# VachaLab/gorder

Measured on AMD Instinct MI355X. Metric: trajectory frames/sec, higher is better.
Workload: dtype f32

## Files before the change

gorder_amd/csrc/gorder_hip.hip:

```cpp
#include <hip/hip_runtime.h>

#include <dlfcn.h>

#include <cmath>
#include <cstdio>
#include <cstdlib>
#include <cstring>
#include <mutex>
#include <new>
#include <string>
#include <deque>
#include <vector>

#include "../../include/gorder_hip.h"
#include "gm_math.h"
#include "plan.h"

#pragma clang fp contract(off)

using gorder::DirectItem;
using gorder::Item;
using gorder::kBlock;
using gorder::Plan;
using gorder::Tile;
// ... 1004 lines not shown
            for (uint32_t k = 0; k < mt.n_molecules; k++) {
                const uint32_t hd = mt.heads ? mt.heads[k] : 0;
                if (hd >= t->n_atoms) return fail(h, GORDER_ERR_INVALID_ARGUMENT, "head index out of range");
                heads.push_back(hd);
                if (lf.method == GORDER_LEAFLETS_INDIVIDUAL)
                    for (uint32_t q = 0; q < mt.n_methyls; q++) {
                        const uint32_t a = mt.methyls[(size_t)k * mt.n_methyls + q];
                        if (a >= t->n_atoms) return fail(h, GORDER_ERR_INVALID_ARGUMENT, "methyl index out of range");
                        ma.push_back(a);
                    }
                mb.push_back((uint32_t)ma.size());
            }
        }
        if ((st = upload(h, &h->d_heads, heads)) != GORDER_OK) return st;
        h->host_heads = heads;
        if (lf.method == GORDER_LEAFLETS_LOCAL) {
            std::vector<uint32_t> ms;
            for (uint32_t m = 0; m < t->n_molecule_types; m++) ms.insert(ms.end(), t->molecule_types[m].n_molecules, p.slot0[m]);
            if ((st = upload(h, &h->d_mol_slot0, ms)) != GORDER_OK) return st;
        }
        if ((st = upload(h, &h->d_methyl_begin, mb)) != GORDER_OK) return st;
        if ((st = upload(h, &h->d_methyl_atoms, ma)) != GORDER_OK) return st;
        if (lf.method == GORDER_LEAFLETS_LOCAL && !(lf.radius > 0.0f))
            return fail(h, GORDER_ERR_INVALID_ARGUMENT, "local leaflets need a positive radius");
        if (lf.method == GORDER_LEAFLETS_GLOBAL || lf.method == GORDER_LEAFLETS_LOCAL) {
            if (!lf.membrane || lf.n_membrane == 0)
                return fail(h, GORDER_ERR_INVALID_ARGUMENT, "global/local leaflets need the membrane group");
            std::vector<uint32_t> mem(lf.membrane, lf.membrane + lf.n_membrane);
            for (uint32_t a : mem)
                if (a >= t->n_atoms) return fail(h, GORDER_ERR_INVALID_ARGUMENT, "membrane index out of range");
            if ((st = upload(h, &h->d_membrane, mem)) != GORDER_OK) return st;
            h->membrane_is_frame = lf.n_membrane == t->n_atoms && !env_flag("GORDER_HIP_LEAFLETS_GENERIC");
            for (uint32_t i = 0; i < lf.n_membrane && h->membrane_is_frame; i++) h->membrane_is_frame = mem[i] == i;
        }
        if (lf.method == GORDER_LEAFLETS_GLOBAL && p.spec_ok && !env_flag("GORDER_HIP_NO_SPECULATE")) {
            std::vector<uint2> own(p.tiles.size());
            for (size_t i = 0; i < own.size(); i++) own[i] = make_uint2(p.own[2 * i], p.own[2 * i + 1]);
            if ((st = upload(h, &h->d_own, own)) != GORDER_OK) return st;
            std::vector<std::vector<SpecSample>> per_mol(p.n_mol_total);
            for (const Tile &tile : p.tiles)
                for (uint32_t q = 0; q < tile.n_items; q++) {
                    const Item &it = p.items[tile.item0 + q];
                    per_mol[it.mol].push_back({tile.atom0 + it.li, tile.atom0 + it.lj, p.tile_slots[tile.slot0 + it.lslot]});
                }
            std::vector<uint32_t> mbeg(1, 0);
            std::vector<SpecSample> all;
            for (const auto &v : per_mol) { all.insert(all.end(), v.begin(), v.end()); mbeg.push_back((uint32_t)all.size()); }
            if ((st = upload(h, &h->d_spec_mol_begin, mbeg)) != GORDER_OK) return st;
            if ((st = upload(h, &h->d_spec_samples, all)) != GORDER_OK) return st;
            std::vector<uint2> oh(p.own_heads.size() / 2);
            for (size_t i = 0; i < oh.size(); i++) oh[i] = make_uint2(p.own_heads[2 * i], p.own_heads[2 * i + 1]);
            if ((st = upload(h, &h->d_own_head_begin, p.own_head_begin)) != GORDER_OK) return st;
            if ((st = upload(h, &h->d_own_heads, oh)) != GORDER_OK) return st;
            HIP_TRY(h, hipMalloc((void **)&h->d_spec_counters, 4 * sizeof(uint32_t)));
            HIP_TRY(h, hipMemset(h->d_spec_counters, 0, 4 * sizeof(uint32_t)));
            HIP_TRY(h, hipHostMalloc((void **)&h->h_spec_counters, 2 * gorder_hip_handle::kSpecRing * sizeof(uint32_t)));
            for (hipEvent_t &ev : h->spec_counters_copied) HIP_TRY(h, hipEventCreateWithFlags(&ev, hipEventDisableTiming));
            h->spec_enabled = true;
        }
        if (lf.method == GORDER_LEAFLETS_LOCAL) {
            const size_t nm = lf.n_membrane, ncell = (size_t)kLocalMaxCells1D * kLocalMaxCells1D;
            const size_t sl = h->local_slab = local_slab_frames(nm);
            for (const void *fn : {reinterpret_cast<const void *>(k_local_build<2>), reinterpret_cast<const void *>(k_local_build<5>),
                                   reinterpret_cast<const void *>(k_local_build<kLocalBuildTrips>)})
                HIP_TRY(h, hipFuncSetAttribute(fn, hipFuncAttributeMaxDynamicSharedMemorySize, (int)kLocalBuildLds));
            h->local_halo = t->handle_pbc && !env_flag("GORDER_HIP_LOCAL_ATOMS_ONLY");
            h->local_rec_stride = (h->local_halo ? 2u : 1u) * nm;
            HIP_TRY(h, hipMalloc((void **)&h->d_lcell_of, sl * nm * sizeof(uint32_t)));
            HIP_TRY(h, hipMalloc((void **)&h->d_ltrig, sl * h->local_rec_stride * sizeof(LocalRec)));
            HIP_TRY(h, hipMalloc((void **)&h->d_lcell_count, sl * (ncell + 1) * sizeof(uint32_t)));
            HIP_TRY(h, hipMalloc((void **)&h->d_lcell_fill, sl * ncell * sizeof(uint32_t)));
            HIP_TRY(h, hipMalloc((void **)&h->d_lgrid, sl * sizeof(uint4)));
            if (h->local_halo) {
                HIP_TRY(h, hipMalloc((void **)&h->d_lrowpre, sl * (size_t)kLocalMaxCells1D * (kLocalMaxCells1D + 1u) * sizeof(LocalRowPre)));
                HIP_TRY(h, hipMalloc((void **)&h->d_ledge, sl * (size_t)kLocalMaxCells1D * (kLocalMaxCells1D + 1u) * sizeof(LocalEdge)));
                HIP_TRY(h, hipMalloc((void **)&h->d_lfinfo, sl * sizeof(float4)));
                HIP_TRY(h, hipMalloc((void **)&h->d_lneed, (sl + 1) * sizeof(uint32_t)));
                HIP_TRY(h, hipMalloc((void **)&h->d_lsummary, 2 * sizeof(uint32_t)));
                HIP_TRY(h, hipMemset(h->d_lsummary, 0, 2 * sizeof(uint32_t)));
                HIP_TRY(h, hipHostMalloc((void **)&h->h_lsummary, 2 * sizeof(uint32_t)));
                h->h_lsummary[0] = h->h_lsummary[1] = 0u;
                HIP_TRY(h, hipEventCreateWithFlags(&h->lsummary_written, hipEventDisableTiming));
                HIP_TRY(h, hipFuncSetAttribute(reinterpret_cast<const void *>(k_local_decide), hipFuncAttributeMaxDynamicSharedMemorySize,
                                               (int)kDecideLds));
                HIP_TRY(h, hipFuncSetAttribute(reinterpret_cast<const void *>(k_local_sums), hipFuncAttributeMaxDynamicSharedMemorySize,
                                               (int)kSumsLds));
                HIP_TRY(h, hipMalloc((void **)&h->d_ltodo, (1 + sl * (size_t)(p.n_mol_total ? p.n_mol_total : 1)) * sizeof(uint2)));
            }
        }
        HIP_TRY(h, hipMalloc((void **)&h->d_adist, sizeof(float) * (p.n_mol_total ? p.n_mol_total : 1)));
    }
    HIP_TRY(h, hipDeviceSynchronize());
    return GORDER_OK;
}

void gorder_hip_destroy(gorder_hip_handle *h) {
    if (!h) return;
    (void)hipSetDevice(h->device);
    if (h->stream) (void)hipStreamSynchronize(h->stream);
    if (h->traj_cache_free) h->traj_cache_free(h);
    for (hipEvent_t ev : h->timing_ev)
        if (ev) (void)hipEventDestroy(ev);
    (void)hipFree(h->d_mol_slot0);
    (void)hipFree(h->d_tiles); (void)hipFree(h->d_items); (void)hipFree(h->d_tile_slots);
    (void)hipFree(h->d_direct); (void)hipFree(h->d_err); (void)hipFree(h->d_xtc_cp);
    (void)hipFree(h->d_ua_tiles); (void)hipFree(h->d_ua_items); (void)hipFree(h->d_ua_tile_slots);
    (void)hipFree(h->d_map_sums); (void)hipFree(h->d_map_cnts); (void)hipFree(h->d_map_packed); (void)hipFree(h->d_tw_sums); (void)hipFree(h->d_tw_cnts);
    (void)hipFree(h->d_geom_group); (void)hipFree(h->d_shapes); (void)hipFree(h->d_inv_box);
// ... 38 lines not shown
    h->stream = hip_stream ? (hipStream_t)hip_stream : h->own_stream;
    return GORDER_OK;
}

static void spec_poll(gorder_hip_handle *h, bool wait);
int gorder_hip_speculation_stats(gorder_hip_handle *h, uint64_t out[4]) {
    if (!h || !out) return GORDER_ERR_INVALID_ARGUMENT;
    HIP_TRY(h, hipSetDevice(h->device));
    HIP_TRY(h, hipStreamSynchronize(h->stream));
    spec_poll(h, true);
    out[0] = h->spec_batches; out[1] = h->spec_fixed; out[2] = h->spec_exact_frames; out[3] = h->spec_enabled ? 1 : 0;
    return GORDER_OK;
}

int gorder_hip_local_decide_stats(gorder_hip_handle *h, uint64_t out[4]) {
    if (!h || !out) return GORDER_ERR_INVALID_ARGUMENT;
    HIP_TRY(h, hipSetDevice(h->device));
    HIP_TRY(h, hipStreamSynchronize(h->stream));
    out[0] = h->decide_submits; out[1] = h->decide_paused_submits;
    out[2] = h->h_lsummary ? h->h_lsummary[0] : 0; out[3] = h->h_lsummary ? h->h_lsummary[1] : 0;
    return GORDER_OK;
}

int gorder_hip_plan(const gorder_hip_handle *h, gorder_hip_plan_t *plan) {
    if (!h || !plan) return GORDER_ERR_INVALID_ARGUMENT;
    plan->n_tiles = (uint32_t)h->plan.tiles.size();
    plan->block_threads = kBlock;
    plan->max_window_atoms = h->plan.max_window;
    plan->n_direct_items = (uint32_t)h->plan.direct.size();
    plan->frames_per_stage = (uint32_t)h->frames_per_stage;
    plan->lds_bytes = (uint32_t)h->lds_bytes;
    plan->map_staged = h->map_staged ? 1u : 0u;
    plan->map_lds_bytes = (uint32_t)h->map_lds_bytes;
    plan->leaflets_one_read = h->plan.spec_ok ? 1u : 0u;
    return GORDER_OK;
}

static void spec_poll(gorder_hip_handle *h, bool wait) {
    for (uint32_t i = 0; i < gorder_hip_handle::kSpecRing; i++) {
        if (!h->spec_ring_frames[i]) continue;
        if (wait) (void)hipEventSynchronize(h->spec_counters_copied[i]);
        else if (hipEventQuery(h->spec_counters_copied[i]) != hipSuccess) continue;
        const uint32_t moved = h->h_spec_counters[2 * i], exact = h->h_spec_counters[2 * i + 1];
        h->spec_fixed += moved;
        h->spec_exact_frames += exact;
        if ((uint64_t)exact * 8u > h->spec_ring_frames[i] ||
            (uint64_t)moved * 16u > h->spec_ring_frames[i] * h->plan.n_mol_total)
            h->spec_enabled = false;
        h->spec_ring_frames[i] = 0;
    }
}

static int run_leaflets(gorder_hip_handle *h, const float *d_xyz, const float *d_box,
                        const std::vector<uint32_t> &aframes, uint32_t row0, const uint8_t *skip = nullptr) {
    if (aframes.empty()) return GORDER_OK;
    int st;
    const size_t cap_before = h->aframes_cap;
    if ((st = ensure(h, &h->d_aframes, &h->aframes_cap, aframes.size())) != GORDER_OK) return st;
    if (h->aframes_cap != cap_before) h->up_aframes_at = nullptr;
    if (h->up_aframes_at != h->d_aframes || h->up_aframes != aframes) {
        HIP_TRY(h, hipMemcpyAsync(h->d_aframes, aframes.data(), aframes.size() * sizeof(uint32_t),
                                  hipMemcpyHostToDevice, h->stream));
        h->up_aframes = aframes;
        h->up_aframes_at = h->d_aframes;
    }
    const gorder_leaflets_t &lf = h->tables.leaflets;
    LeafletArgs la{};
    la.xyz = d_xyz; la.box9 = d_box; la.n_atoms = h->plan.n_atoms;
    la.aframes = h->d_aframes; la.row0 = row0; la.aflags = h->d_aflags; la.adist = h->d_adist;
    la.n_mol_total = h->plan.n_mol_total; la.heads = h->d_heads;
    la.membrane = h->d_membrane; la.n_membrane = lf.n_membrane;
    la.methyl_begin = h->d_methyl_begin; la.methyl_atoms = h->d_methyl_atoms;
    la.dim = lf.normal_dim; la.flip = lf.flip ? 1 : 0; la.pbc = h->tables.handle_pbc ? 1 : 0;
    la.err = h->d_err;
    la.skip = skip;
    la.n_assign = (uint32_t)aframes.size();
    if (lf.method == GORDER_LEAFLETS_GLOBAL) {
        const dim3 g(skip ? std::min<uint32_t>((uint32_t)aframes.size(), 512u) : (uint32_t)aframes.size()), b(1024);
        TIMING_MARK(h, h->membrane_is_frame ? "k_leaflets_global_contig" : "k_leaflets_global");
        if (h->membrane_is_frame) {
            if (skip) hipLaunchKernelGGL(k_leaflets_global_contig<true>, g, dim3(256), 0, h->stream, la);
            else hipLaunchKernelGGL(k_leaflets_global_contig<false>, g, dim3(256), 0, h->stream, la);
        } else {
            if (skip) hipLaunchKernelGGL(k_leaflets_global<true>, g, b, 0, h->stream, la);
            else hipLaunchKernelGGL(k_leaflets_global<false>, g, b, 0, h->stream, la);
        }
    } else if (lf.method == GORDER_LEAFLETS_INDIVIDUAL) {
        TIMING_MARK(h, "k_leaflets_individual");
        size_t done = 0;
        while (done < aframes.size()) {
            const uint32_t ny = (uint32_t)std::min<size_t>(aframes.size() - done, 65535);
            LeafletArgs lb = la;
            lb.aframes = h->d_aframes + done;
            lb.row0 = row0 + (uint32_t)done;
            if (done + ny < aframes.size()) lb.adist = nullptr;
            hipLaunchKernelGGL(k_leaflets_individual, dim3((la.n_mol_total + 255) / 256, ny), dim3(256), 0,
                               h->stream, lb);
            done += ny;
        }
    }
    else if (lf.method == GORDER_LEAFLETS_LOCAL) {
        const size_t ncell = (size_t)kLocalMaxCells1D * kLocalMaxCells1D;
        LocalArgs lo{};
        lo.xyz = d_xyz; lo.box9 = d_box; lo.n_atoms = h->plan.n_atoms;
        lo.aflags = h->d_aflags; lo.adist = h->d_adist; lo.n_mol_total = h->plan.n_mol_total;
        lo.heads = h->d_heads; lo.mol_slot0 = h->d_mol_slot0; lo.n_membrane = lf.n_membrane;
        lo.membrane = h->membrane_is_frame ? nullptr : h->d_membrane;
        lo.dim = lf.normal_dim; lo.flip = lf.flip ? 1 : 0; lo.pbc = h->tables.handle_pbc ? 1 : 0;
        lo.radius = lf.radius;
        lo.radius_thr = local_radius_threshold(lf.radius);
        lo.cell_of = h->d_lcell_of; lo.trig = h->d_ltrig; lo.cell_count = h->d_lcell_count;
        lo.cell_fill = h->d_lcell_fill; lo.err = h->d_err;
        lo.grid = h->d_lgrid;
        lo.halo = h->local_halo ? 1 : 0;
        lo.prune = env_flag("GORDER_HIP_LOCAL_NO_PRUNE") ? 0 : (env_flag("GORDER_HIP_LOCAL_DECIDE_NOTHING") ? 2 : 1);
        lo.rec_stride = (uint32_t)h->local_rec_stride;
        lo.rowpre = h->d_lrowpre;
        lo.edge = h->d_ledge;
        lo.finfo = h->d_lfinfo;
        lo.todo = h->d_ltodo;
        bool decide = lo.halo && lo.prune && lo.n_mol_total && !env_flag("GORDER_HIP_LOCAL_NO_DECIDE");
        if (decide) {
            if (h->lsummary_pending) {
                if (hipEventQuery(h->lsummary_written) == hipSuccess) {
                    h->lsummary_pending = false;
                    if (2u * h->h_lsummary[0] > h->h_lsummary[1]) h->decide_pause = gorder_hip_handle::kDecidePause;
                } else {
                    (void)hipGetLastError();
// ... 145 lines not shown
        HIP_TRY(h, hipMemsetAsync(nc, 0, ncap * row * sizeof(unsigned long long), h->stream));
        if (h->d_tw_sums) {
            HIP_TRY(h, hipMemcpyAsync(ns, h->d_tw_sums, h->n_frames * row * sizeof(unsigned long long), hipMemcpyDeviceToDevice, h->stream));
            HIP_TRY(h, hipMemcpyAsync(nc, h->d_tw_cnts, h->n_frames * row * sizeof(unsigned long long), hipMemcpyDeviceToDevice, h->stream));
            HIP_TRY(h, hipStreamSynchronize(h->stream));
            HIP_TRY(h, hipFree(h->d_tw_sums));
            HIP_TRY(h, hipFree(h->d_tw_cnts));
        }
        h->d_tw_sums = ns; h->d_tw_cnts = nc; h->tw_cap = ncap;
    }
    FrameArgs a{};
    a.xyz = d_xyz; a.box9 = d_box; a.n_atoms = p.n_atoms; a.n_frames = n_frames;
    a.pbc = pbc ? 1 : 0;
    a.nx = h->tables.normal[0]; a.ny = h->tables.normal[1]; a.nz = h->tables.normal[2]; a.n2 = h->n2; a.n2sq = h->n2sq;
    a.leaflets = leaflets ? 1 : 0; a.aflags = h->d_aflags; a.arow = h->d_arow; a.n_mol_total = p.n_mol_total;
    a.acc = h->d_acc; a.rep = h->d_rep; a.n_rep = h->n_rep; a.n_acc = p.n_acc; a.err = h->d_err;
    h->manual_active = false;
    if (h->manual_frames) {
        const size_t n4 = (size_t)n_frames * p.n_mol_total;
        if ((st = ensure(h, &h->d_dyn_normals, &h->dyn_normals_cap, n4)) != GORDER_OK) return abort_batch(st);
        if (hipStreamSynchronize(h->stream) != hipSuccess ||
            hipMemcpy(h->d_dyn_normals, h->manual_normals.data(), n4 * 4 * sizeof(float), hipMemcpyHostToDevice) != hipSuccess)
            return abort_batch(fail(h, GORDER_ERR_DEVICE, "manual normals: copy to the device failed"));
        h->manual_active = true;
        h->manual_frames = 0;
    }
    const uint32_t n_tiles_all = (uint32_t)p.tiles.size();
    if (spec) {
        if ((st = ensure(h, &h->d_mom, &h->mom_cap, (size_t)n_frames * n_tiles_all)) != GORDER_OK) return abort_batch(st);
        if ((st = ensure(h, &h->d_head_z, &h->head_z_cap, (size_t)n_frames * p.n_mol_total)) != GORDER_OK) return abort_batch(st);
        a.own = h->d_own; a.mom = h->d_mom; a.mom_dim = (int)lf.normal_dim;
        a.own_head_begin = h->d_own_head_begin; a.own_heads = h->d_own_heads; a.head_z = h->d_head_z;
        h->spec_now = true;
    }
    st = launch_orders(h, a);
    h->spec_now = false;
    h->manual_active = false;
    if (st != GORDER_OK) return abort_batch(st);
    h->rep_dirty = true;
    if (spec) {
        size_t cap_c = h->spec_frames_cap, cap_o = h->spec_frames_cap;
        if ((st = ensure(h, &h->d_spec_center, &cap_c, n_frames)) != GORDER_OK) return abort_batch(st);
        if ((st = ensure(h, &h->d_spec_ok, &cap_o, n_frames)) != GORDER_OK) return abort_batch(st);
        h->spec_frames_cap = std::min(cap_c, cap_o);
        uint32_t *cnt = h->d_spec_counters + 2u * (uint32_t)(h->spec_batches & 1u);
        uint32_t *cnt_next = h->d_spec_counters + 2u * (uint32_t)((h->spec_batches + 1u) & 1u);
        SpecArgs sa{};
        sa.xyz = d_xyz; sa.box9 = d_box; sa.n_atoms = p.n_atoms; sa.n_frames = n_frames; sa.n_tiles = n_tiles_all;
        sa.n_mol_total = p.n_mol_total; sa.n_membrane = lf.n_membrane; sa.dim = lf.normal_dim; sa.flip = lf.flip ? 1 : 0;
        sa.pbc = pbc ? 1 : 0; sa.mom = h->d_mom; sa.head_z = h->d_head_z; sa.center = h->d_spec_center; sa.ok = h->d_spec_ok;
        sa.aflags = h->d_aflags; sa.adist = h->d_adist; sa.counters = cnt; sa.counters_next = cnt_next;
        const uint32_t ring_slot = (uint32_t)(h->spec_batches % gorder_hip_handle::kSpecRing);
        sa.host_counters = h->h_spec_counters + 2u * ring_slot; sa.err = h->d_err;
        (void)timing_mark(h, "k_spec_check + k_spec_fixup");
        hipLaunchKernelGGL(k_spec_check, dim3(std::min<uint32_t>(n_frames, 2048u)), dim3(256), 0, h->stream, sa);
        if ((st = run_leaflets(h, d_xyz, d_box, spec_aframes, 1, h->d_spec_ok)) != GORDER_OK) return abort_batch(st);
        (void)timing_mark(h, "k_spec_check + k_spec_fixup");
        const uint32_t fix_grid = (uint32_t)std::min<uint64_t>(((uint64_t)n_frames * p.n_mol_total + 63u) / 64u, 4096u);
        if (h->extra.tw)
            hipLaunchKernelGGL((k_spec_fixup<false, true>), dim3(fix_grid), dim3(64), 0, h->stream, a, sa, h->d_spec_mol_begin,
                               h->d_spec_samples, h->d_tw_sums, h->d_tw_cnts, (uint64_t)h->n_frames);
        else if (h->tables.flags & GORDER_FLAG_TRIG_ACOS_COS)
            hipLaunchKernelGGL((k_spec_fixup<true, false>), dim3(fix_grid), dim3(64), 0, h->stream, a, sa, h->d_spec_mol_begin,
                               h->d_spec_samples, (unsigned long long *)nullptr, (unsigned long long *)nullptr, (uint64_t)0);
        else
            hipLaunchKernelGGL((k_spec_fixup<false, false>), dim3(fix_grid), dim3(64), 0, h->stream, a, sa, h->d_spec_mol_begin,
                               h->d_spec_samples, (unsigned long long *)nullptr, (unsigned long long *)nullptr, (uint64_t)0);
        hipLaunchKernelGGL(k_spec_finish, dim3(1), dim3(256), 0, h->stream, sa);
        HIP_TRY(h, hipGetLastError());
        HIP_TRY(h, hipEventRecord(h->spec_counters_copied[ring_slot], h->stream));
        h->spec_ring_frames[ring_slot] = n_frames;
        h->spec_batches++;
    }
    if (n_new_rows) {
        HIP_TRY(h, hipMemcpyAsync(h->d_aflags, h->d_aflags + n_new_rows * (size_t)p.n_mol_total, p.n_mol_total,
                                  hipMemcpyDeviceToDevice, h->stream));
    }
    {
        gorder_hip_handle::BatchLog rec{h->n_submits, frame_index[0], n_frames > 1 ? frame_index[1] - frame_index[0] : 0, {}};
        for (uint32_t f = 1; f < n_frames; f++)
            if (frame_index[f] != rec.first + (uint64_t)f * rec.stride) { rec.list.assign(frame_index, frame_index + n_frames); break; }
        if (h->batch_log.size() >= gorder_hip_handle::kBatchLog) h->batch_log.pop_front();
        h->batch_log.push_back(std::move(rec));
        TIMING_MARK(h, "k_batch_end");
        hipLaunchKernelGGL(k_batch_end, dim3(pbc ? std::min<uint32_t>((n_frames + 255u) / 256u, 256u) : 1u), dim3(256), 0, h->stream,
                           pbc ? d_box : nullptr, n_frames, h->d_err,
                           h->d_acc + 4 * (size_t)p.n_acc, (unsigned long long)h->n_submits, h->decoder_key);
        HIP_TRY(h, hipGetLastError());
        TIMING_MARK(h, nullptr);
        if (h->timing_on) h->timing_launches++;
        h->n_submits++;
    }
    h->n_frames += n_frames;
    return GORDER_OK;
}

int gorder_hip_submit_host(gorder_hip_handle *h, const float *xyz, const float *box, const uint64_t *frame_index,
                           uint32_t n_frames) {
    if (!h || !xyz || !frame_index) return GORDER_ERR_INVALID_ARGUMENT;
    if (n_frames == 0) return GORDER_OK;
    HIP_TRY(h, hipSetDevice(h->device));
    int st;
    const size_t nx = (size_t)n_frames * h->plan.n_atoms * 3u, nb = (size_t)n_frames * 9u;
    if (!h->copy_stream) {
        HIP_TRY(h, hipStreamCreateWithFlags(&h->copy_stream, hipStreamNonBlocking));
        for (int k = 0; k < 2; k++) {
            HIP_TRY(h, hipEventCreateWithFlags(&h->stage_copied[k], hipEventDisableTiming));
            HIP_TRY(h, hipEventCreateWithFlags(&h->stage_computed[k], hipEventDisableTiming));
        }
    }
    const int b = h->stage_next;
    h->stage_next ^= 1;
    if (h->stage_used[b]) HIP_TRY(h, hipEventSynchronize(h->stage_computed[b]));
    if ((st = ensure(h, &h->d_stage_xyz[b], &h->stage_xyz_cap[b], nx)) != GORDER_OK) return st;
    HIP_TRY(h, hipMemcpyAsync(h->d_stage_xyz[b], xyz, nx * sizeof(float), hipMemcpyHostToDevice, h->copy_stream));
    if (box) {
        if ((st = ensure(h, &h->d_stage_box[b], &h->stage_box_cap[b], nb)) != GORDER_OK) return st;
        HIP_TRY(h, hipMemcpyAsync(h->d_stage_box[b], box, nb * sizeof(float), hipMemcpyHostToDevice, h->copy_stream));
    }
    HIP_TRY(h, hipEventRecord(h->stage_copied[b], h->copy_stream));
    HIP_TRY(h, hipStreamWaitEvent(h->stream, h->stage_copied[b], 0));
// ... 180 lines not shown
    HIP_TRY(h, hipMemcpyAsync(d_sums, h->d_map_sums, n * sizeof(unsigned long long), hipMemcpyDeviceToDevice, h->stream));
    HIP_TRY(h, hipMemcpyAsync(d_counts, h->d_map_cnts, n * sizeof(unsigned long long), hipMemcpyDeviceToDevice, h->stream));
    HIP_TRY(h, hipStreamSynchronize(h->stream));
    return check_device_error(h);
}

int gorder_hip_bind_accumulators(gorder_hip_handle *h, void *d_ptr, uint64_t n_u64) {
    if (!h || !d_ptr || n_u64 < h->acc_words || ((uintptr_t)d_ptr & 7u)) return GORDER_ERR_INVALID_ARGUMENT;
    HIP_TRY(h, hipSetDevice(h->device));
    {
        const int st = fold_replicas(h);
        if (st != GORDER_OK) return st;
    }
    HIP_TRY(h, hipMemcpyAsync(d_ptr, h->d_acc, h->acc_words * sizeof(unsigned long long), hipMemcpyDeviceToDevice, h->stream));
    HIP_TRY(h, hipStreamSynchronize(h->stream));
    if (!h->acc_external) HIP_TRY(h, hipFree(h->d_acc));
    h->d_acc = (unsigned long long *)d_ptr;
    h->acc_external = true;
    return GORDER_OK;
}

int gorder_hip_reset(gorder_hip_handle *h) {
    if (!h) return GORDER_ERR_INVALID_ARGUMENT;
    HIP_TRY(h, hipSetDevice(h->device));
    const Plan &p = h->plan;
    HIP_TRY(h, hipMemsetAsync(h->d_acc, 0, h->acc_words * sizeof(unsigned long long), h->stream));
    if (h->d_rep) HIP_TRY(h, hipMemsetAsync(h->d_rep, 0, (size_t)h->n_rep * 4u * p.n_acc * sizeof(unsigned long long), h->stream));
    h->rep_dirty = false;
    if (h->extra.maps) {
        const size_t nmap = 3 * (size_t)p.n_acc * h->map_nx * h->map_ny;
        const size_t npk = (h->tables.leaflets.method != GORDER_LEAFLETS_NONE ? 2 : 1) * (nmap / 3);
        HIP_TRY(h, hipMemsetAsync(h->d_map_sums, 0, nmap * sizeof(unsigned long long), h->stream));
        HIP_TRY(h, hipMemsetAsync(h->d_map_cnts, 0, nmap * sizeof(unsigned long long), h->stream));
        HIP_TRY(h, hipMemsetAsync(h->d_map_packed, 0, npk * sizeof(unsigned long long), h->stream));
        h->map_pending = 0;
    }
    if (h->d_tw_sums) {
        const size_t n = h->tw_cap * 3 * (size_t)p.n_acc * sizeof(unsigned long long);
        HIP_TRY(h, hipMemsetAsync(h->d_tw_sums, 0, n, h->stream));
        HIP_TRY(h, hipMemsetAsync(h->d_tw_cnts, 0, n, h->stream));
    }
    HIP_TRY(h, hipMemsetAsync(h->d_err, 0xff, kErrWords * sizeof(uint32_t), h->stream));
    h->batch_log.clear();
    h->n_frames = 0;
    h->have_assignment = false;
    h->assignment_frame = 0;
    h->manual_frames = 0;
    h->err_index = 0;
    h->err_msg.clear();
    if (h->d_own) {
        spec_poll(h, true);
        h->spec_enabled = true;
        h->spec_batches = h->spec_fixed = h->spec_exact_frames = 0;
        HIP_TRY(h, hipMemsetAsync(h->d_spec_counters, 0, 4 * sizeof(uint32_t), h->stream));
    }
    if (h->d_lsummary) {
        if (h->lsummary_pending) { (void)hipEventSynchronize(h->lsummary_written); h->lsummary_pending = false; }
        h->decide_pause = 0;
        h->decide_submits = h->decide_paused_submits = 0;
        h->h_lsummary[0] = h->h_lsummary[1] = 0u;
        HIP_TRY(h, hipMemsetAsync(h->d_lsummary, 0, 2 * sizeof(uint32_t), h->stream));
    }
    return GORDER_OK;
}

int gorder_hip_comm_unique_id(uint8_t id[128]) {
    if (!id) return GORDER_ERR_INVALID_ARGUMENT;
    RcclApi *api = rccl_api(nullptr);
    if (!api) return GORDER_ERR_DEVICE;
    UniqueId u;
    if (api->get_unique_id(&u) != 0) return GORDER_ERR_DEVICE;
    memcpy(id, u.internal, 128);
    return GORDER_OK;
}

int gorder_hip_comm_create(gorder_hip_handle *h, const uint8_t id[128], int n_ranks, int rank, void **comm_out) {
    if (!h || !id || !comm_out || n_ranks < 1 || rank < 0 || rank >= n_ranks) return GORDER_ERR_INVALID_ARGUMENT;
    *comm_out = nullptr;
    std::string why;
    RcclApi *api = rccl_api(&why);
    if (!api) return fail(h, GORDER_ERR_DEVICE, why);
    HIP_TRY(h, hipSetDevice(h->device));
    UniqueId u;
    memcpy(u.internal, id, 128);
    const int rc = api->comm_init_rank(comm_out, n_ranks, u, rank);
    if (rc != 0) return fail(h, GORDER_ERR_DEVICE, rccl_error(api, "ncclCommInitRank", rc));
    return GORDER_OK;
}

void gorder_hip_comm_destroy(void *comm) {
    RcclApi *api = rccl_api(nullptr);
    if (api && comm) (void)api->comm_destroy(comm);
}

int gorder_hip_allreduce(gorder_hip_handle *h, void *nccl_comm) {
    if (!h || !nccl_comm) return GORDER_ERR_INVALID_ARGUMENT;
    std::string why;
    RcclApi *api = rccl_api(&why);
    if (!api) return fail(h, GORDER_ERR_DEVICE, why);
    HIP_TRY(h, hipSetDevice(h->device));
    int st = fold_replicas(h);
    if (st != GORDER_OK) return st;
    if ((st = fold_maps(h)) != GORDER_OK) return st;
    int rc = api->group_start();
    if (rc == 0) rc = api->all_reduce(h->d_acc, h->d_acc, h->acc_words, kNcclInt64, kNcclSum, nccl_comm, h->stream);
    if (rc == 0 && h->extra.maps) {
        const size_t nmap = 3 * (size_t)h->plan.n_acc * h->map_nx * h->map_ny;
// ... 90 lines not shown
```

gorder_amd/csrc/kernels_leaflets.h:

```cpp
#pragma once

namespace {

struct LeafletArgs {
    const float *xyz;
    const float *box9;
    uint32_t n_atoms;
    const uint32_t *aframes;
    uint32_t row0;
    uint8_t *aflags;
    float *adist;
    uint32_t n_mol_total;
    const uint32_t *heads;
    const uint32_t *membrane;
    uint32_t n_membrane;
    const uint32_t *methyl_begin;
    const uint32_t *methyl_atoms;
    uint32_t dim;
    int flip, pbc;
    uint32_t *err;
    const uint8_t *skip;
    uint32_t n_assign;
};

__device__ __forceinline__ void fast_sincos_rev(float u, float *sn, float *cs);
__device__ __forceinline__ void local_trig(float z, float inv_L, float *sn, float *cs) {
    fast_sincos_rev(z * inv_L, sn, cs);
}
__device__ __forceinline__ void fast_sincos_rev(float u, float *sn, float *cs) {
    *sn = __builtin_amdgcn_sinf(u);
    *cs = __builtin_amdgcn_cosf(u);
}

__device__ __forceinline__ double wave_sum(double v) {
    for (int off = 32; off > 0; off >>= 1) v += __shfl_xor(v, off, 64);
    return v;
}

__device__ __forceinline__ double block_sum(double v, double *scratch) {
    v = wave_sum(v);
    const uint32_t wave = threadIdx.x >> 6, n_waves = (blockDim.x + 63u) >> 6;
    if ((threadIdx.x & 63u) == 0) scratch[wave] = v;
    __syncthreads();
    double r = 0.0;
    for (uint32_t w = 0; w < n_waves; w++) r += scratch[w];
    __syncthreads();
    return r;
}

__device__ __forceinline__ void block_sum2(double &v0, double &v1, double *scratch) {
    v0 = wave_sum(v0);
    v1 = wave_sum(v1);
    const uint32_t wave = threadIdx.x >> 6, n_waves = (blockDim.x + 63u) >> 6;
    if ((threadIdx.x & 63u) == 0) { scratch[wave] = v0; scratch[16 + wave] = v1; }
    __syncthreads();
    double r0 = 0.0, r1 = 0.0;
    for (uint32_t w = 0; w < n_waves; w++) { r0 += scratch[w]; r1 += scratch[16 + w]; }
    __syncthreads();
    v0 = r0; v1 = r1;
}

struct GeomArgs {
    const float *xyz;
    const float *box9;
    uint32_t n_atoms;
    int pbc;
    uint32_t kind, reference, orientation;
    float point[3];
    const uint32_t *group;
    uint32_t n_group;
    float xdim[2], ydim[2], zdim[2], radius, span[2], structure_box[3];
    float *shapes;
    uint32_t *err;
};

// ... 109 lines not shown
            float sn, cs;
            fast_sincos_rev(gm_wrap(dn == 0 ? px : (dn == 1 ? py : pz), L, bad) * inv, &sn, &cs);
            sc += cs;
            ss += sn;
        }
    }
    if (a.pbc) {
        const double tc = block_sum((double)sc, scratch), ts = block_sum((double)ss, scratch);
        est = (atan2f(-(float)ts, -(float)tc) + 3.1415927f) / (6.2831855f / L);
    }
    float acc = 0.0f;
#pragma unroll
    for (int k = 0; k < KEEP; k++) {
        const uint32_t i = threadIdx.x + (uint32_t)k * nthr;
        if (i < a.n_membrane) {
            const float dx = keep[k] - est;
            acc += a.pbc ? gm_min_image(dx, L, bad) : dx;
        }
    }
    for (uint32_t i = threadIdx.x + (uint32_t)KEEP * nthr; i < a.n_membrane; i += nthr) {
        const float dx = x[3u * (size_t)a.membrane[i] + dn] - est;
        acc += a.pbc ? gm_min_image(dx, L, bad) : dx;
    }
    const double tot = block_sum((double)acc, scratch);
    const double nf = block_sum((double)nonfinite, scratch);
    if (threadIdx.x == 0) {
        float c = est + (float)(tot / (double)a.n_membrane);
        if (a.pbc) c = gm_wrap(c, L, bad);
        if (c != c || nf != 0.0 || a.n_membrane == 0) {
            raise_error(a.err, GORDER_ERR_INVALID_GLOBAL_MEMBRANE_CENTER, f, kStageSystem);
            c = __builtin_nanf("");
        }
        s_center = c;
    }
    __syncthreads();
    const float cdim = s_center;
    uint8_t *row = a.aflags + (size_t)(a.row0 + bi) * a.n_mol_total;
    const bool last = bi + 1 == a.n_assign;
    for (uint32_t m = threadIdx.x; m < a.n_mol_total; m += blockDim.x) {
        const float hp = x[3u * (size_t)a.heads[m] + dn];
        float d = hp - cdim;
        if (a.pbc) d = gm_min_image(d, L, bad);
        row[m] = (uint8_t)((d >= 0.0f ? 0 : 1) ^ (a.flip ? 1 : 0));
        if (last && a.adist) a.adist[m] = d;
    }
    if (bad) raise_box_range(a.err, f);
}
template <bool TURNS>
__global__ __launch_bounds__(1024) void k_leaflets_global(LeafletArgs a) {
    if (!TURNS) {
        leaflets_global_frame(a, blockIdx.x);
        return;
    }
    for (uint32_t bi = blockIdx.x; bi < a.n_assign; bi += gridDim.x) {
        leaflets_global_frame(a, bi);
        __syncthreads();
    }
}

__device__ __forceinline__ void block_minmax(float &lo, float &hi, float *scratch ) {
    for (int off = 32; off > 0; off >>= 1) {
        lo = fminf(lo, __shfl_xor(lo, off, 64));
        hi = fmaxf(hi, __shfl_xor(hi, off, 64));
    }
    const uint32_t wave = threadIdx.x >> 6, n_waves = (blockDim.x + 63u) >> 6;
    if ((threadIdx.x & 63u) == 0) { scratch[wave] = lo; scratch[16 + wave] = hi; }
    __syncthreads();
    for (uint32_t w = 0; w < n_waves; w++) { lo = fminf(lo, scratch[w]); hi = fmaxf(hi, scratch[16 + w]); }
    __syncthreads();
}

__device__ __forceinline__ void leaflets_global_contig_frame(const LeafletArgs &a, uint32_t bi) {
    __shared__ double scratch[32];
    __shared__ float fscratch[32];
    __shared__ float s_center;
    const uint32_t f = a.aframes[bi];
    if (a.skip && a.skip[f]) return;
    const uint32_t dn = a.dim;
    float L = 1.0f;
    if (a.pbc) L = a.box9[9 * (size_t)f + 4 * dn];
    int bad = 0;
    const size_t start = (size_t)f * a.n_atoms * 3u;
    const uint32_t sh = (uint32_t)(start & 3u), n_float = 3u * a.n_atoms;
    const uint32_t n4 = (sh + n_float + 3u) >> 2;
    const v4f *src = reinterpret_cast<const v4f *>(a.xyz + (start - sh));
    const float *x = a.xyz + start;
    const bool pbc = a.pbc != 0;
    const float inv = pbc ? 1.0f / L : 0.0f;
    const float zref = a.n_mol_total ? x[3u * (size_t)a.heads[0] + dn] : 0.0f;
    uint32_t r = (dn + sh + 3u * 256u - threadIdx.x) % 3u;
    float nonfinite = 0.0f, sc = 0.0f, ss = 0.0f, su = 0.0f, ulo = 3.0e38f, uhi = -3.0e38f;
    auto take = [&](float z, bool ok) {
        z = ok ? z : zref;
        if (pbc) {
            bad |= (ok && !(z <= 9.0f * L && z >= -8.0f * L)) ? 1 : 0;
            float sn, cs;
            fast_sincos_rev(z * inv, &sn, &cs);
            sc += ok ? cs : 0.0f;
            ss += ok ? sn : 0.0f;
        }
        const float u = pbc ? gm_min_image(z - zref, L, bad) : z - zref;
        su += ok ? u : 0.0f;
        ulo = ok ? fminf(ulo, u) : ulo;
        uhi = ok ? fmaxf(uhi, u) : uhi;
    };
    auto chunk = [&](const v4f v, uint32_t c, uint32_t j0) {
// ... 63 lines not shown
    block_minmax(ulo, uhi, fscratch);
    float center;
    if (!pbc) {
        center = zref + (float)(tu / (double)a.n_atoms);
    } else {
        const float est = (atan2f(-(float)ts, -(float)tc) + 3.1415927f) / (6.2831855f / L);
        const float shift = gm_min_image(zref - est, L, bad);
        const float half = L / 2.0f, margin = 1e-4f * L;
        if (ulo + shift > -half + margin && uhi + shift < half - margin) {
            center = gm_wrap((est + shift) + (float)(tu / (double)a.n_atoms), L, bad);
        } else {
            float acc = 0.0f;
            uint32_t r2 = (dn + sh + 3u * 256u - threadIdx.x) % 3u;
            for (uint32_t c2 = threadIdx.x; c2 < n4; c2 += 256u) {
                const v4f v = src[c2];
                const uint32_t e0 = 4u * c2, j0 = r2;
                float za = v.x;
                za = j0 == 1 ? v.y : za;
                za = j0 == 2 ? v.z : za;
                if (e0 + j0 >= sh && e0 + j0 < sh + n_float) acc += gm_min_image(za - est, L, bad);
                if (j0 == 0 && e0 + 3u >= sh && e0 + 3u < sh + n_float) acc += gm_min_image(v.w - est, L, bad);
                r2 = r2 == 0 ? 2u : r2 - 1u;
            }
            const double tot = block_sum((double)acc, scratch);
            center = gm_wrap(est + (float)(tot / (double)a.n_atoms), L, bad);
        }
    }
    if (threadIdx.x == 0) {
        if (center != center || nf != 0.0 || a.n_atoms == 0) {
            raise_error(a.err, GORDER_ERR_INVALID_GLOBAL_MEMBRANE_CENTER, f, kStageSystem);
            center = __builtin_nanf("");
        }
        s_center = center;
    }
    __syncthreads();
    const float cdim = s_center;
    uint8_t *row = a.aflags + (size_t)(a.row0 + bi) * a.n_mol_total;
    const bool last = bi + 1 == a.n_assign;
    for (uint32_t m = threadIdx.x; m < a.n_mol_total; m += blockDim.x) {
        const float hp = x[3u * (size_t)a.heads[m] + dn];
        float d = hp - cdim;
        if (pbc) d = gm_min_image(d, L, bad);
        row[m] = (uint8_t)((d >= 0.0f ? 0 : 1) ^ (a.flip ? 1 : 0));
        if (last && a.adist) a.adist[m] = d;
    }
    if (bad) raise_box_range(a.err, f);
}
template <bool TURNS>
__global__ __launch_bounds__(256) void k_leaflets_global_contig(LeafletArgs a) {
    if (!TURNS) {
        leaflets_global_contig_frame(a, blockIdx.x);
        return;
    }
    for (uint32_t bi = blockIdx.x; bi < a.n_assign; bi += gridDim.x) {
        leaflets_global_contig_frame(a, bi);
        __syncthreads();
    }
}

struct SpecArgs {
    const float *xyz;
    const float *box9;
    uint32_t n_atoms, n_frames, n_tiles, n_mol_total, n_membrane;
    uint32_t dim;
    int flip, pbc;
    const float4 *mom;
    const float *head_z;
    float *center;
    uint8_t *ok;
    uint8_t *aflags;
    float *adist;
    uint32_t *counters;
    uint32_t *counters_next;
    uint32_t *host_counters;
    uint32_t *err;
};
__global__ __launch_bounds__(256) void k_spec_check(SpecArgs a) {
    __shared__ float s_center;
    __shared__ int s_ok;
    for (uint32_t f = blockIdx.x; f < a.n_frames; f += gridDim.x) {
        const float L = a.pbc ? a.box9[9 * (size_t)f + 4 * a.dim] : 0.0f;
        if (threadIdx.x < 64u) {
            double S = 0.0, Q = 0.0;
            float mn = 3.0e38f, mx = -3.0e38f;
            for (uint32_t t = threadIdx.x; t < a.n_tiles; t += 64u) {
                const float4 m = a.mom[(size_t)f * a.n_tiles + t];
                S += (double)m.x; Q += (double)m.y;
                mn = fminf(mn, m.z); mx = fmaxf(mx, m.w);
            }
            for (int off = 32; off >= 1; off >>= 1) {
                S += __shfl_xor(S, off, 64); Q += __shfl_xor(Q, off, 64);
                mn = fminf(mn, __shfl_xor(mn, off, 64)); mx = fmaxf(mx, __shfl_xor(mx, off, 64));
            }
            if (threadIdx.x == 0u) {
                const double n = (double)a.n_membrane, c = S / n;
                bool ok = (S - S == 0.0) && (Q - Q == 0.0) && mn <= mx;
                if (ok && a.pbc) {
                    const double k = 6.283185307179586 / (double)L;
                    const double var = fmax(Q - S * S / n, 0.0) + 1e-4 * Q + 1e-6 * n;
                    const double dmax = k * fmax((double)mx - c, c - (double)mn), S2 = k * k * var, den = n - 0.5 * S2;
                    ok = den > 0.0 && L > 0.0f;
                    if (ok) {
                        const double dist = (dmax * S2 / 6.0 / den) / k;
                        const double room = 0.5 * (double)L - 1e-4 * (double)L - dist;
                        ok = (double)mx - c < room && c - (double)mn < room;
                    }
                }
                a.center[f] = (float)c;
                a.ok[f] = ok ? 1 : 0;
                s_center = (float)c;
                s_ok = ok ? 1 : 0;
                if (!ok) atomicAdd(&a.counters[1], 1u);
            }
        }
        __syncthreads();
        if (s_ok) {
            const float c = s_center;
            const bool last = f + 1 == a.n_frames;
            int bad = 0;
            for (uint32_t m = threadIdx.x; m < a.n_mol_total; m += blockDim.x) {
                float d = a.head_z[(size_t)f * a.n_mol_total + m] - c;
                if (a.pbc) d = gm_min_image(d, L, bad);
                a.aflags[(size_t)(1u + f) * a.n_mol_total + m] = (uint8_t)((d >= 0.0f ? 0 : 1) ^ (a.flip ? 1 : 0));
                if (last && a.adist) a.adist[m] = d;
            }
            if (bad) raise_box_range(a.err, f);
        }
        __syncthreads();
    }
}
struct SpecSample { uint32_t i, j, slot; };
template <bool ACOS_COS, bool TW>
__global__ __launch_bounds__(64) void k_spec_fixup(FrameArgs a, SpecArgs sa, const uint32_t *__restrict__ mol_begin,
                                                   const SpecSample *__restrict__ samples, unsigned long long *tw_sums,
                                                   unsigned long long *tw_cnts, uint64_t tw_row0) {
    const uint64_t n_pairs = (uint64_t)sa.n_frames * sa.n_mol_total;
    uint32_t moved = 0;
    for (uint64_t p0 = (uint64_t)blockIdx.x * 64u; p0 < n_pairs; p0 += (uint64_t)gridDim.x * 64u) {
        const uint64_t pi = p0 + threadIdx.x;
        bool differs = false;
        uint32_t exact_l = 0;
        if (pi < n_pairs) {
            exact_l = sa.aflags[(size_t)sa.n_mol_total + pi];
            differs = exact_l != sa.aflags[pi % sa.n_mol_total];
        }
        unsigned long long todo = __ballot(differs);
        moved += (uint32_t)__popcll(todo);
        while (todo) {
            const int l = __ffsll((long long)todo) - 1;
            todo &= todo - 1ull;
            const uint64_t pj = p0 + (uint64_t)l;
            const uint32_t f = (uint32_t)(pj / sa.n_mol_total), m = (uint32_t)(pj - (uint64_t)f * sa.n_mol_total);
            const uint32_t exact = (uint32_t)__shfl((int)exact_l, l, 64);
            const float *x = a.xyz + (size_t)f * a.n_atoms * 3u;
            for (uint32_t q = mol_begin[m] + threadIdx.x; q < mol_begin[m + 1]; q += 64u) {
                const SpecSample sm = samples[q];
                SampleAcc acc;
                int bad = 0;
                const float *p1 = x + 3u * (size_t)sm.i, *p2 = x + 3u * (size_t)sm.j;
                bond_sample<ACOS_COS>(a, f, p1[0], p1[1], p1[2], p2[0], p2[1], p2[2], m, acc, bad);
                unsigned long long *rep = a.rep;
                if (exact == 0u) {
                    atomicAdd(&rep[(size_t)a.n_acc + sm.slot], (unsigned long long)acc.s_tot);
                    atomicAdd(&rep[3u * (size_t)a.n_acc + sm.slot], 1ull);
                } else {
                    atomicAdd(&rep[(size_t)a.n_acc + sm.slot], (unsigned long long)(-acc.s_tot));
                    atomicAdd(&rep[3u * (size_t)a.n_acc + sm.slot], ~0ull);
                }
                if (TW) {
                    const size_t up = (size_t)(tw_row0 + f) * 3u * a.n_acc + (size_t)a.n_acc + sm.slot;
                    atomicAdd(&tw_sums[up], (unsigned long long)(exact == 0u ? acc.s_tot : -acc.s_tot));
                    atomicAdd(&tw_cnts[up], exact == 0u ? 1ull : ~0ull);
                }
            }
        }
    }
    if (threadIdx.x == 0u && moved) atomicAdd(&sa.counters[0], moved);
}
__global__ __launch_bounds__(256) void k_spec_finish(SpecArgs sa) {
    for (uint32_t m = threadIdx.x; m < sa.n_mol_total; m += blockDim.x)
        sa.aflags[m] = sa.aflags[(size_t)sa.n_frames * sa.n_mol_total + m];
    if (threadIdx.x == 0u) {
        sa.host_counters[0] = sa.counters[0];
        sa.host_counters[1] = sa.counters[1];
        sa.counters_next[0] = 0u;
        sa.counters_next[1] = 0u;
    }
}

__global__ __launch_bounds__(256) void k_leaflets_individual(LeafletArgs a) {
    const uint32_t m = blockIdx.x * blockDim.x + threadIdx.x;
    if (m >= a.n_mol_total) return;
    const uint32_t f = a.aframes[blockIdx.y];
    const float *x = a.xyz + (size_t)f * a.n_atoms * 3u;
    float L = 1.0f;
    if (a.pbc) L = a.box9[9 * (size_t)f + 4 * a.dim];
    int bad = 0;
    const float hp = x[3u * (size_t)a.heads[m] + a.dim];
    float total = 0.0f;
    for (uint32_t k = a.methyl_begin[m]; k < a.methyl_begin[m + 1]; k++) {
        const float mp = x[3u * (size_t)a.methyl_atoms[k] + a.dim];
        const float d = hp - mp;
        total += a.pbc ? gm_min_image(d, L, bad) : d;
    }
    a.aflags[(size_t)(a.row0 + blockIdx.y) * a.n_mol_total + m] =
        (uint8_t)((total >= 0.0f ? 0 : 1) ^ (a.flip ? 1 : 0));
    if (blockIdx.y + 1 == gridDim.y && a.adist) a.adist[m] = total;
    if (bad) raise_box_range(a.err, f);
}

constexpr uint32_t kLocalMaxCells1D = 128;
constexpr uint32_t kLocalSlabMax = 2048;
inline uint32_t local_slab_frames(size_t n_membrane) {
    const size_t per_frame = n_membrane * (2u * 12u + 4u) + (size_t)(2 * 4u + 16u + 16u) * kLocalMaxCells1D * (kLocalMaxCells1D + 1u) + 32u;
    const size_t n = ((size_t)4096 << 20) / per_frame;
    uint32_t cap = kLocalSlabMax;
    if (const char *ev = getenv("GORDER_HIP_LOCAL_SLAB")) cap = (uint32_t)std::max(4, atoi(ev));
    return (uint32_t)(n < 4 ? 4 : (n > cap ? cap : n));
}

struct LocalRowPre { float sc, ss; double sz; };
struct alignas(16) LocalEdge { uint32_t q; float zm, sq; uint32_t cs; };
constexpr uint32_t kEdgeSpanMax = 2000;
__device__ __forceinline__ uint32_t local_edge_trig(float sc, float ss) {
    return ((uint32_t)(int)__builtin_rintf(sc * 16.0f) & 0xffffu) | ((uint32_t)(int)__builtin_rintf(ss * 16.0f) << 16);
}
__device__ __forceinline__ void local_edge_trig_diff(uint32_t hi, uint32_t lo, float &dc, float &ds) {
    dc = (float)(int16_t)((hi & 0xffffu) - (lo & 0xffffu)) * 0.0625f;
    ds = (float)(int16_t)((hi >> 16) - (lo >> 16)) * 0.0625f;
}
struct LocalRec { float x, y, z; };

struct LocalArgs {
    const float *xyz;
    const float *box9;
    uint32_t n_atoms;
    const uint32_t *aframes;
// ... 1403 lines not shown
```

Measured before the change: 20.79 million.

## Fuse speculative leaflet fixup into check kernel and drop finish launch

The speculative leaflet path now performs bond re-sampling for molecules that changed leaflet directly inside the check kernel for frames whose speculation was validated. The fixup kernel handles only frames that failed the check, and it does so only when the exact-frame counter is nonzero. The separate finish kernel is folded into fixup through a last-block ticket counter. Leaflet-global kernels skip their work when no frames need exact assignment. This removes launches and full-pass scans, at the cost of a small fixed fixup grid and added ticket synchronisation.

```diff
diff --git a/gorder_amd/csrc/gorder_hip.hip b/gorder_amd/csrc/gorder_hip.hip
--- a/gorder_amd/csrc/gorder_hip.hip
+++ b/gorder_amd/csrc/gorder_hip.hip
@@ -1080,8 +1080,8 @@
             for (size_t i = 0; i < oh.size(); i++) oh[i] = make_uint2(p.own_heads[2 * i], p.own_heads[2 * i + 1]);
             if ((st = upload(h, &h->d_own_head_begin, p.own_head_begin)) != GORDER_OK) return st;
             if ((st = upload(h, &h->d_own_heads, oh)) != GORDER_OK) return st;
-            HIP_TRY(h, hipMalloc((void **)&h->d_spec_counters, 4 * sizeof(uint32_t)));
-            HIP_TRY(h, hipMemset(h->d_spec_counters, 0, 4 * sizeof(uint32_t)));
+            HIP_TRY(h, hipMalloc((void **)&h->d_spec_counters, 5 * sizeof(uint32_t)));
+            HIP_TRY(h, hipMemset(h->d_spec_counters, 0, 5 * sizeof(uint32_t)));
             HIP_TRY(h, hipHostMalloc((void **)&h->h_spec_counters, 2 * gorder_hip_handle::kSpecRing * sizeof(uint32_t)));
             for (hipEvent_t &ev : h->spec_counters_copied) HIP_TRY(h, hipEventCreateWithFlags(&ev, hipEventDisableTiming));
             h->spec_enabled = true;
@@ -1226,7 +1226,8 @@
 }
 
 static int run_leaflets(gorder_hip_handle *h, const float *d_xyz, const float *d_box,
-                        const std::vector<uint32_t> &aframes, uint32_t row0, const uint8_t *skip = nullptr) {
+                        const std::vector<uint32_t> &aframes, uint32_t row0, const uint8_t *skip = nullptr,
+                        const uint32_t *n_left = nullptr) {
     if (aframes.empty()) return GORDER_OK;
     int st;
     const size_t cap_before = h->aframes_cap;
@@ -1248,6 +1249,7 @@
     la.dim = lf.normal_dim; la.flip = lf.flip ? 1 : 0; la.pbc = h->tables.handle_pbc ? 1 : 0;
     la.err = h->d_err;
     la.skip = skip;
+    la.n_left = n_left;
     la.n_assign = (uint32_t)aframes.size();
     if (lf.method == GORDER_LEAFLETS_GLOBAL) {
         const dim3 g(skip ? std::min<uint32_t>((uint32_t)aframes.size(), 512u) : (uint32_t)aframes.size()), b(1024);
@@ -1499,21 +1501,26 @@
         sa.aflags = h->d_aflags; sa.adist = h->d_adist; sa.counters = cnt; sa.counters_next = cnt_next;
         const uint32_t ring_slot = (uint32_t)(h->spec_batches % gorder_hip_handle::kSpecRing);
         sa.host_counters = h->h_spec_counters + 2u * ring_slot; sa.err = h->d_err;
+        sa.ticket = h->d_spec_counters + 4u;
+        sa.mol_begin = h->d_spec_mol_begin; sa.samples = h->d_spec_samples;
+        sa.tw_sums = h->d_tw_sums; sa.tw_cnts = h->d_tw_cnts; sa.tw_row0 = h->n_frames;
+        const uint32_t check_grid = std::min<uint32_t>(n_frames, 2048u);
+        const uint32_t fix_grid = (uint32_t)std::min<uint64_t>(((uint64_t)n_frames * p.n_mol_total + 255u) / 256u, 8u);
         (void)timing_mark(h, "k_spec_check + k_spec_fixup");
-        hipLaunchKernelGGL(k_spec_check, dim3(std::min<uint32_t>(n_frames, 2048u)), dim3(256), 0, h->stream, sa);
-        if ((st = run_leaflets(h, d_xyz, d_box, spec_aframes, 1, h->d_spec_ok)) != GORDER_OK) return abort_batch(st);
+        if (h->extra.tw)
+            hipLaunchKernelGGL((k_spec_check<false, true>), dim3(check_grid), dim3(256), 0, h->stream, a, sa);
+        else if (h->tables.flags & GORDER_FLAG_TRIG_ACOS_COS)
+            hipLaunchKernelGGL((k_spec_check<true, false>), dim3(check_grid), dim3(256), 0, h->stream, a, sa);
+        else
+            hipLaunchKernelGGL((k_spec_check<false, false>), dim3(check_grid), dim3(256), 0, h->stream, a, sa);
+        if ((st = run_leaflets(h, d_xyz, d_box, spec_aframes, 1, h->d_spec_ok, cnt + 1)) != GORDER_OK) return abort_batch(st);
         (void)timing_mark(h, "k_spec_check + k_spec_fixup");
-        const uint32_t fix_grid = (uint32_t)std::min<uint64_t>(((uint64_t)n_frames * p.n_mol_total + 63u) / 64u, 4096u);
         if (h->extra.tw)
-            hipLaunchKernelGGL((k_spec_fixup<false, true>), dim3(fix_grid), dim3(64), 0, h->stream, a, sa, h->d_spec_mol_begin,
-                               h->d_spec_samples, h->d_tw_sums, h->d_tw_cnts, (uint64_t)h->n_frames);
+            hipLaunchKernelGGL((k_spec_fixup<false, true>), dim3(fix_grid), dim3(256), 0, h->stream, a, sa);
         else if (h->tables.flags & GORDER_FLAG_TRIG_ACOS_COS)
-            hipLaunchKernelGGL((k_spec_fixup<true, false>), dim3(fix_grid), dim3(64), 0, h->stream, a, sa, h->d_spec_mol_begin,
-                               h->d_spec_samples, (unsigned long long *)nullptr, (unsigned long long *)nullptr, (uint64_t)0);
+            hipLaunchKernelGGL((k_spec_fixup<true, false>), dim3(fix_grid), dim3(256), 0, h->stream, a, sa);
         else
-            hipLaunchKernelGGL((k_spec_fixup<false, false>), dim3(fix_grid), dim3(64), 0, h->stream, a, sa, h->d_spec_mol_begin,
-                               h->d_spec_samples, (unsigned long long *)nullptr, (unsigned long long *)nullptr, (uint64_t)0);
-        hipLaunchKernelGGL(k_spec_finish, dim3(1), dim3(256), 0, h->stream, sa);
+            hipLaunchKernelGGL((k_spec_fixup<false, false>), dim3(fix_grid), dim3(256), 0, h->stream, a, sa);
         HIP_TRY(h, hipGetLastError());
         HIP_TRY(h, hipEventRecord(h->spec_counters_copied[ring_slot], h->stream));
         h->spec_ring_frames[ring_slot] = n_frames;
@@ -1800,7 +1807,7 @@
         spec_poll(h, true);
         h->spec_enabled = true;
         h->spec_batches = h->spec_fixed = h->spec_exact_frames = 0;
-        HIP_TRY(h, hipMemsetAsync(h->d_spec_counters, 0, 4 * sizeof(uint32_t), h->stream));
+        HIP_TRY(h, hipMemsetAsync(h->d_spec_counters, 0, 5 * sizeof(uint32_t), h->stream));
     }
     if (h->d_lsummary) {
         if (h->lsummary_pending) { (void)hipEventSynchronize(h->lsummary_written); h->lsummary_pending = false; }
diff --git a/gorder_amd/csrc/kernels_leaflets.h b/gorder_amd/csrc/kernels_leaflets.h
--- a/gorder_amd/csrc/kernels_leaflets.h
+++ b/gorder_amd/csrc/kernels_leaflets.h
@@ -21,6 +21,7 @@
     uint32_t *err;
     const uint8_t *skip;
     uint32_t n_assign;
+    const uint32_t *n_left;
 };
 
 __device__ __forceinline__ void fast_sincos_rev(float u, float *sn, float *cs);
@@ -236,6 +237,7 @@
         leaflets_global_frame(a, blockIdx.x);
         return;
     }
+    if (a.n_left && *a.n_left == 0u) return;
     for (uint32_t bi = blockIdx.x; bi < a.n_assign; bi += gridDim.x) {
         leaflets_global_frame(a, bi);
         __syncthreads();
@@ -405,12 +407,14 @@
         leaflets_global_contig_frame(a, blockIdx.x);
         return;
     }
+    if (a.n_left && *a.n_left == 0u) return;
     for (uint32_t bi = blockIdx.x; bi < a.n_assign; bi += gridDim.x) {
         leaflets_global_contig_frame(a, bi);
         __syncthreads();
     }
 }
 
+struct SpecSample { uint32_t i, j, slot; };
 struct SpecArgs {
     const float *xyz;
     const float *box9;
@@ -426,11 +430,57 @@
     uint32_t *counters;
     uint32_t *counters_next;
     uint32_t *host_counters;
+    uint32_t *ticket;
     uint32_t *err;
+    const uint32_t *mol_begin;
+    const SpecSample *samples;
+    unsigned long long *tw_sums, *tw_cnts;
+    uint64_t tw_row0;
 };
-__global__ __launch_bounds__(256) void k_spec_check(SpecArgs a) {
+template <bool ACOS_COS, bool TW>
+__device__ __forceinline__ void spec_move_pair(const FrameArgs &a, const SpecArgs &sa, uint32_t f, uint32_t m, uint32_t exact) {
+    const uint32_t lane = threadIdx.x & 63u;
+    const float *x = a.xyz + (size_t)f * a.n_atoms * 3u;
+    for (uint32_t q = sa.mol_begin[m] + lane; q < sa.mol_begin[m + 1]; q += 64u) {
+        const SpecSample sm = sa.samples[q];
+        SampleAcc acc;
+        int bad = 0;
+        const float *p1 = x + 3u * (size_t)sm.i, *p2 = x + 3u * (size_t)sm.j;
+        bond_sample<ACOS_COS>(a, f, p1[0], p1[1], p1[2], p2[0], p2[1], p2[2], m, acc, bad);
+        unsigned long long *rep = a.rep;
+        if (exact == 0u) {
+            atomicAdd(&rep[(size_t)a.n_acc + sm.slot], (unsigned long long)acc.s_tot);
+            atomicAdd(&rep[3u * (size_t)a.n_acc + sm.slot], 1ull);
+        } else {
+            atomicAdd(&rep[(size_t)a.n_acc + sm.slot], (unsigned long long)(-acc.s_tot));
+            atomicAdd(&rep[3u * (size_t)a.n_acc + sm.slot], ~0ull);
+        }
+        if (TW) {
+            const size_t up = (size_t)(sa.tw_row0 + f) * 3u * a.n_acc + (size_t)a.n_acc + sm.slot;
+            atomicAdd(&sa.tw_sums[up], (unsigned long long)(exact == 0u ? acc.s_tot : -acc.s_tot));
+            atomicAdd(&sa.tw_cnts[up], exact == 0u ? 1ull : ~0ull);
+        }
+    }
+}
+template <bool ACOS_COS, bool TW>
+__device__ __forceinline__ uint32_t spec_move_pairs(const FrameArgs &a, const SpecArgs &sa, uint64_t p0, bool differs, uint32_t exact_l) {
+    unsigned long long todo = __ballot(differs);
+    const uint32_t moved = (uint32_t)__popcll(todo);
+    while (todo) {
+        const int l = __ffsll((long long)todo) - 1;
+        todo &= todo - 1ull;
+        const uint64_t pj = p0 + (uint64_t)l;
+        const uint32_t f = (uint32_t)(pj / sa.n_mol_total), m = (uint32_t)(pj - (uint64_t)f * sa.n_mol_total);
+        const uint32_t exact = (uint32_t)__shfl((int)exact_l, l, 64);
+        spec_move_pair<ACOS_COS, TW>(a, sa, f, m, exact);
+    }
+    return moved;
+}
+template <bool ACOS_COS, bool TW>
+__global__ __launch_bounds__(256) void k_spec_check(FrameArgs fa, SpecArgs a) {
     __shared__ float s_center;
     __shared__ int s_ok;
+    uint32_t moved = 0;
     for (uint32_t f = blockIdx.x; f < a.n_frames; f += gridDim.x) {
         const float L = a.pbc ? a.box9[9 * (size_t)f + 4 * a.dim] : 0.0f;
         if (threadIdx.x < 64u) {
@@ -471,71 +521,59 @@
             const float c = s_center;
             const bool last = f + 1 == a.n_frames;
             int bad = 0;
-            for (uint32_t m = threadIdx.x; m < a.n_mol_total; m += blockDim.x) {
-                float d = a.head_z[(size_t)f * a.n_mol_total + m] - c;
-                if (a.pbc) d = gm_min_image(d, L, bad);
-                a.aflags[(size_t)(1u + f) * a.n_mol_total + m] = (uint8_t)((d >= 0.0f ? 0 : 1) ^ (a.flip ? 1 : 0));
-                if (last && a.adist) a.adist[m] = d;
+            const uint32_t lane = threadIdx.x & 63u;
+            for (uint32_t m0 = threadIdx.x - lane; m0 < a.n_mol_total; m0 += blockDim.x) {
+                const uint32_t m = m0 + lane;
+                bool differs = false;
+                uint32_t side = 0;
+                if (m < a.n_mol_total) {
+                    float d = a.head_z[(size_t)f * a.n_mol_total + m] - c;
+                    if (a.pbc) d = gm_min_image(d, L, bad);
+                    side = (d >= 0.0f ? 0u : 1u) ^ (a.flip ? 1u : 0u);
+                    a.aflags[(size_t)(1u + f) * a.n_mol_total + m] = (uint8_t)side;
+                    differs = side != a.aflags[m];
+                    if (last && a.adist) a.adist[m] = d;
+                }
+                moved += spec_move_pairs<ACOS_COS, TW>(fa, a, (uint64_t)f * a.n_mol_total + m0, differs, side);
             }
             if (bad) raise_box_range(a.err, f);
         }
         __syncthreads();
     }
-}
-struct SpecSample { uint32_t i, j, slot; };
+    if ((threadIdx.x & 63u) == 0u && moved) atomicAdd(&a.counters[0], moved);
+}
 template <bool ACOS_COS, bool TW>
-__global__ __launch_bounds__(64) void k_spec_fixup(FrameArgs a, SpecArgs sa, const uint32_t *__restrict__ mol_begin,
-                                                   const SpecSample *__restrict__ samples, unsigned long long *tw_sums,
-                                                   unsigned long long *tw_cnts, uint64_t tw_row0) {
+__global__ __launch_bounds__(256) void k_spec_fixup(FrameArgs a, SpecArgs sa) {
+    __shared__ uint32_t l_last;
     const uint64_t n_pairs = (uint64_t)sa.n_frames * sa.n_mol_total;
     uint32_t moved = 0;
-    for (uint64_t p0 = (uint64_t)blockIdx.x * 64u; p0 < n_pairs; p0 += (uint64_t)gridDim.x * 64u) {
-        const uint64_t pi = p0 + threadIdx.x;
-        bool differs = false;
-        uint32_t exact_l = 0;
-        if (pi < n_pairs) {
-            exact_l = sa.aflags[(size_t)sa.n_mol_total + pi];
-            differs = exact_l != sa.aflags[pi % sa.n_mol_total];
-        }
-        unsigned long long todo = __ballot(differs);
-        moved += (uint32_t)__popcll(todo);
-        while (todo) {
-            const int l = __ffsll((long long)todo) - 1;
-            todo &= todo - 1ull;
-            const uint64_t pj = p0 + (uint64_t)l;
-            const uint32_t f = (uint32_t)(pj / sa.n_mol_total), m = (uint32_t)(pj - (uint64_t)f * sa.n_mol_total);
-            const uint32_t exact = (uint32_t)__shfl((int)exact_l, l, 64);
-            const float *x = a.xyz + (size_t)f * a.n_atoms * 3u;
-            for (uint32_t q = mol_begin[m] + threadIdx.x; q < mol_begin[m + 1]; q += 64u) {
-                const SpecSample sm = samples[q];
-                SampleAcc acc;
-                int bad = 0;
-                const float *p1 = x + 3u * (size_t)sm.i, *p2 = x + 3u * (size_t)sm.j;
-                bond_sample<ACOS_COS>(a, f, p1[0], p1[1], p1[2], p2[0], p2[1], p2[2], m, acc, bad);
-                unsigned long long *rep = a.rep;
-                if (exact == 0u) {
-                    atomicAdd(&rep[(size_t)a.n_acc + sm.slot], (unsigned long long)acc.s_tot);
-                    atomicAdd(&rep[3u * (size_t)a.n_acc + sm.slot], 1ull);
-                } else {
-                    atomicAdd(&rep[(size_t)a.n_acc + sm.slot], (unsigned long long)(-acc.s_tot));
-                    atomicAdd(&rep[3u * (size_t)a.n_acc + sm.slot], ~0ull);
-                }
-                if (TW) {
-                    const size_t up = (size_t)(tw_row0 + f) * 3u * a.n_acc + (size_t)a.n_acc + sm.slot;
-                    atomicAdd(&tw_sums[up], (unsigned long long)(exact == 0u ? acc.s_tot : -acc.s_tot));
-                    atomicAdd(&tw_cnts[up], exact == 0u ? 1ull : ~0ull);
-                }
-            }
-        }
-    }
-    if (threadIdx.x == 0u && moved) atomicAdd(&sa.counters[0], moved);
-}
-__global__ __launch_bounds__(256) void k_spec_finish(SpecArgs sa) {
+    if (*(volatile const uint32_t *)&sa.counters[1] != 0u) {
+        const uint32_t lane = threadIdx.x & 63u;
+        const uint64_t step = (uint64_t)gridDim.x * blockDim.x;
+        for (uint64_t p0 = (uint64_t)blockIdx.x * blockDim.x + (threadIdx.x - lane); p0 < n_pairs; p0 += step) {
+            const uint64_t pi = p0 + lane;
+            bool differs = false;
+            uint32_t exact_l = 0;
+            if (pi < n_pairs && !sa.ok[pi / sa.n_mol_total]) {
+                exact_l = sa.aflags[(size_t)sa.n_mol_total + pi];
+                differs = exact_l != sa.aflags[pi % sa.n_mol_total];
+            }
+            moved += spec_move_pairs<ACOS_COS, TW>(a, sa, p0, differs, exact_l);
+        }
+        if (lane == 0u && moved) atomicAdd(&sa.counters[0], moved);
+    }
+    __threadfence();
+    __syncthreads();
+    if (threadIdx.x == 0) l_last = atomicAdd(sa.ticket, 1u) == gridDim.x - 1u ? 1u : 0u;
+    __syncthreads();
+    if (!l_last) return;
+    __threadfence();
     for (uint32_t m = threadIdx.x; m < sa.n_mol_total; m += blockDim.x)
         sa.aflags[m] = sa.aflags[(size_t)sa.n_frames * sa.n_mol_total + m];
     if (threadIdx.x == 0u) {
-        sa.host_counters[0] = sa.counters[0];
-        sa.host_counters[1] = sa.counters[1];
+        *sa.ticket = 0u;
+        sa.host_counters[0] = atomicAdd(&sa.counters[0], 0u);
+        sa.host_counters[1] = atomicAdd(&sa.counters[1], 0u);
         sa.counters_next[0] = 0u;
         sa.counters_next[1] = 0u;
     }
```

After: 20.94 million, median of 4. No clear change (+0.8%).
